# keith2018/TinyGPT

Hardware: AMD Instinct MI355X
Metric: decode tokens/sec (and % HBM roofline), Llama-3.2-1B bf16 batch=1, 1 GPU (higher is better)
Workload: dtype bf16; 1 GPU; Llama-3.2-1B bf16, batch 1 per GPU: 2048-token prefill then greedy decode (one step = one token, context 2054..3411); replicas=1, params=1235814400, graph=True

## Files before the change

__graft_entry__.py:

```python
import os
import sys

ROOT = os.path.dirname(os.path.abspath(__file__))
if ROOT not in sys.path:
    sys.path.insert(0, ROOT)


def build() -> None:
    from tinygpt_amd import build as b
    lib = b.build_lib(force=False, verbose=True)
    assert os.path.exists(lib)
    host_lib, cli = b.build_host(force=False, verbose=True)
    assert os.path.exists(host_lib) and os.path.exists(cli)
    b.build_host(force=False, verbose=True, test_hooks=True)
    b.build_kv_pool_check(force=False, verbose=True)
    b.build_splice_plan_check(force=False, verbose=True)
    b.build_dev_mem_check(force=False, verbose=True)
    b.build_row_snapshot_check(force=False, verbose=True)
    b.build_attn_worklist_check(force=False, verbose=True)
    b.build_spec_draft_check(force=False, verbose=True)
    b.build_spec_mode_check(force=False, verbose=True)
    b.build_spec_rows_check(force=False, verbose=True)
    b.build_constraint_check(force=False, verbose=True)
    from oracle.oracle_ffi import build_oracle, oracle_backend
    build_oracle()
    oracle_backend()
    import tinygpt_amd
    from tinygpt_amd.ffi import product_backend
    assert product_backend().abi_version() == 3
    print("build ok:", lib)


def smoke() -> None:
    import json
    os.environ.setdefault("OMP_NUM_THREADS", "8")
    import numpy as np
    from tinygpt_amd.desc import desc_from_hf_config
    from tinygpt_amd.ffi import GREEDY, Model, SamplerCfg, product_backend
    from oracle.oracle_ffi import OracleModel, build_oracle
    build_oracle()
    gd = os.path.join(ROOT, "tests", "golden", "llama_tiny")
    cfg = json.load(open(os.path.join(gd, "config.json")))
    g = np.load(os.path.join(gd, "golden.npz"))
    d = desc_from_hf_config(cfg, "bf16")
    gpu = Model(d, product_backend(), device=0).load_synthetic(int(g["seed"]), float(g["std"])).finalize()
    ref = OracleModel(d).load_synthetic(int(g["seed"]), float(g["std"])).finalize()
    gpu.forward(g["prompt"]); ref.forward(g["prompt"])
    a, b = gpu.logits(rounded=False), ref.logits(rounded=False)
    err = float(np.abs(a - b).max() / np.abs(b).max())
    assert err < 1e-3, f"prefill logits differ from the oracle: rel {err:.3e}"
    tg, tr = gpu.sample(GREEDY), ref.sample(GREEDY)
    dg, dr = gpu.decode(4, GREEDY), ref.decode(4, GREEDY)
# ... 13 lines not shown
```

tinygpt_amd/build.py:

```python
from __future__ import annotations

import os
import shutil
import subprocess
import sys

HERE = os.path.dirname(os.path.abspath(__file__))
CSRC = os.path.join(HERE, "csrc")
LIBDIR = os.path.join(HERE, "lib")
LIB = os.path.join(LIBDIR, "libtgx_mi355x.so")
HIPCC = shutil.which("hipcc") or "/opt/rocm/bin/hipcc"
FLAGS = ["--offload-arch=gfx950", "-O3", "-std=c++17", "-fPIC", "-shared", "-fvisibility=hidden",
         "-Wall", "-Wno-unused-function", "-DNDEBUG",
         ] + (["-mllvm", "-amdgpu-mfma-vgpr-form"] if os.environ.get("TGX_VGPR_FORM", "1") == "1" else [])


TUS = ["abi", "decode", "attn", "sampler", "prefill", "prefill_f32", "skinny"]
OBJDIR = os.path.join(LIBDIR, "obj")


def _deps():
    deps = [os.path.join(HERE, "..", "include", "tgx.h"), os.path.join(CSRC, "ctx.h"), os.path.join(CSRC, "kv_pool.h"), os.path.join(CSRC, "dev_mem.h"), os.path.join(CSRC, "row_snapshot.h"),
            os.path.join(CSRC, "splice_plan.h"), os.path.join(CSRC, "attn_worklist.h"), os.path.join(CSRC, "automaton.h")]
    kd =os.path.join(CSRC, "kernels")
    return deps + [os.path.join(kd, f) for f in sorted(os.listdir(kd))]


def build_lib(force: bool = False, verbose: bool = False, extra_flags=()):
    if os.environ.get("TGX_DISSECT") == "1":
        extra_flags = list(extra_flags) + ["-DTGX_DISSECT=1"]
    if os.environ.get("TGX_EXTRA_FLAGS"):
        extra_flags = list(extra_flags) + os.environ["TGX_EXTRA_FLAGS"].split()
    cflags = [f for f in FLAGS if f != "-shared"] + list(extra_flags)
    stamp, want = LIB + ".flags", " ".join([HIPCC] + cflags)
    same_flags = os.path.exists(stamp) and open(stamp).read() == want
    os.makedirs(OBJDIR, exist_ok=True)
    deps = _deps()
    jobs = []
    for tu in TUS:
        src, obj = os.path.join(CSRC, tu + ".hip"), os.path.join(OBJDIR, tu + ".o")
        fresh = same_flags and os.path.exists(obj) and all(os.path.getmtime(obj) >= os.path.getmtime(d) for d in deps + [src])
        if force or not fresh:
            cmd = [HIPCC] + cflags + ["-c", src, "-o", obj]
            if verbose:
                print(" ".join(cmd), file=sys.stderr)
            jobs.append((tu, subprocess.Popen(cmd)))
    failed = [tu for tu, p in jobs if p.wait() != 0]
    if failed:
        raise subprocess.CalledProcessError(1, "hipcc -c " + ", ".join(failed))
    objs = [os.path.join(OBJDIR, tu + ".o") for tu in TUS]
    if jobs or not os.path.exists(LIB) or any(os.path.getmtime(LIB) < os.path.getmtime(o) for o in objs):
        cmd = [HIPCC, "--offload-arch=gfx950", "-shared", "-fPIC", "-fvisibility=hidden"] + objs + ["-o", LIB]
        if verbose:
            print(" ".join(cmd), file=sys.stderr)
        subprocess.check_call(cmd)
    with open(stamp, "w") as f:
# ... 18 lines not shown
def _build_cpu_check(name, header, force, verbose):
    src, target = os.path.join(HERE, "..", "tests", name + ".cpp"), os.path.join(TEST_BUILD, name)
    os.makedirs(TEST_BUILD, exist_ok=True)
    if force or _stale(target, [src, header]):
        cmd = [CXX, "-std=c++17", "-O1", "-g", "-fsanitize=address,undefined", "-fno-omit-frame-pointer", "-Wall", "-Wextra", src, "-o", target]
        if verbose:
            print(" ".join(cmd), file=sys.stderr)
        subprocess.check_call(cmd)
    return target


def build_kv_pool_check(force: bool = False, verbose: bool = False):
    return _build_cpu_check("kv_pool_check", os.path.join(CSRC, "kv_pool.h"), force, verbose)


def build_splice_plan_check(force: bool = False, verbose: bool = False):
    if _stale(os.path.join(TEST_BUILD, "splice_plan_check"), [os.path.join(CSRC, "kv_pool.h")]):
        force = True
    return _build_cpu_check("splice_plan_check", os.path.join(CSRC, "splice_plan.h"), force, verbose)


def build_dev_mem_check(force: bool = False, verbose: bool = False):
    return _build_cpu_check("dev_mem_check", os.path.join(CSRC, "dev_mem.h"), force, verbose)


def build_row_snapshot_check(force: bool = False, verbose: bool = False):
    return _build_cpu_check("row_snapshot_check", os.path.join(CSRC, "row_snapshot.h"), force, verbose)


def build_attn_worklist_check(force: bool = False, verbose: bool = False):
    return _build_cpu_check("attn_worklist_check", os.path.join(CSRC, "attn_worklist.h"), force, verbose)


def build_spec_draft_check(force: bool = False, verbose: bool = False):
    return _build_cpu_check("spec_draft_check", os.path.join(HOST, "spec_draft.h"), force, verbose)


def build_spec_mode_check(force: bool = False, verbose: bool = False):
    return _build_cpu_check("spec_mode_check", os.path.join(HOST, "spec_mode.h"), force, verbose)


def build_spec_rows_check(force: bool = False, verbose: bool = False):
    return _build_cpu_check("spec_rows_check", os.path.join(HOST, "spec_mode.h"), force, verbose)


def build_constraint_check(force: bool = False, verbose: bool = False):
    if _stale(os.path.join(TEST_BUILD, "constraint_check"), [os.path.join(CSRC, "automaton.h"), os.path.join(HOST, "constraint.h")]):
        force = True
    return _build_cpu_check("constraint_check", os.path.join(HOST, "constraint.cpp"), force, verbose)


def build_host(force: bool = False, verbose: bool = False, test_hooks: bool = False):
    srcs = [os.path.join(HOST, f) for f in ("loader.cpp", "engine.cpp", "regex.cpp", "tokenizer.cpp", "constraint.cpp")]
    deps = [os.path.join(HOST, f) for f in os.listdir(HOST)] + [os.path.join(HERE, "..", "include", "tgx.h"), os.path.join(CSRC, "row_snapshot.h"), os.path.join(CSRC, "automaton.h")]
    lib, cli, flags = HOST_LIB, HOST_CLI, []
    if test_hooks:
        lib, cli, flags = HOST_TEST_LIB, HOST_TEST_CLI, ["-DTGXH_TEST_HOOKS"]
    os.makedirs(os.path.dirname(lib), exist_ok=True)
    for target, extra in ((lib, [os.path.join(HOST, "engine_c.cpp"), "-shared"]), (cli, [os.path.join(HOST, "main.cpp")])):
        if not force and not _stale(target, deps):
            continue
        cmd = [CXX] + CXXFLAGS + flags + srcs + extra + ["-o", target, "-ldl"]
        if verbose:
            print(" ".join(cmd), file=sys.stderr)
        subprocess.check_call(cmd)
    return lib, cli
# ... 7 lines not shown
```

tinygpt_amd/csrc/abi.hip:

```cpp
#include <climits>
#include "ctx.h"
#include "kernels/kv_fork.h"
#include "kernels/kv_pack.h"
#include "kernels/kv_splice.h"
#include "row_snapshot.h"
#include "splice_plan.h"
#include "automaton.h"

static std::string g_create_err;

int set_err(tgx_ctx* c, int code, const char* fmt, ...) {
  char buf[512];
  va_list ap;
  va_start(ap, fmt);
  vsnprintf(buf, sizeof buf, fmt, ap);
  va_end(ap);
  if (c) c->err = buf; else g_create_err = buf;
  return code;
}

namespace {

inline uint16_t host_f32_to_bf16(float f) {
  uint32_t u;
// ... 609 lines not shown
  if (gpt2 && d.qk_norm) return set_err(nullptr, TGX_ERR_INVALID, "gpt2 has no q/k norm");
  if (d.compute_dtype != TGX_BF16 && d.compute_dtype != TGX_F16 && d.compute_dtype != TGX_F32) return set_err(nullptr, TGX_ERR_INVALID, "unknown compute dtype %d", d.compute_dtype);
  if (d.head_dim != 64 && d.head_dim != 128) return set_err(nullptr, TGX_ERR_UNSUPPORTED, "head_dim %d (64 and 128 are built)", d.head_dim);
  if (d.heads <= 0 || d.kv_heads <= 0 || d.heads % d.kv_heads) return set_err(nullptr, TGX_ERR_INVALID, "heads %% kv_heads != 0");
  if (d.heads / d.kv_heads > 16) return set_err(nullptr, TGX_ERR_UNSUPPORTED, "GQA group size %d > 16", d.heads / d.kv_heads);
  if (d.hidden % 8 || d.inter % 8 || (d.heads * d.head_dim) % 8) return set_err(nullptr, TGX_ERR_UNSUPPORTED, "hidden/intermediate sizes must be multiples of 8");
  if (d.hidden <= 0 || d.layers <= 0 || d.inter <= 0 || d.vocab <= 0 || d.max_ctx <= 0) return set_err(nullptr, TGX_ERR_INVALID, "non-positive model dimension");
  if (d.hidden > 16384) return set_err(nullptr, TGX_ERR_UNSUPPORTED, "hidden_size %d > 16384", d.hidden);
  if (d.inter > 65536 || d.heads * d.head_dim > 16384) return set_err(nullptr, TGX_ERR_UNSUPPORTED, "projection input wider than 65536 (intermediate) / 16384 (heads * head_dim)");
  int ndev = 0;
  if (hipGetDeviceCount(&ndev) != hipSuccess || ndev <= 0) return set_err(nullptr, TGX_ERR_DEVICE, "no HIP device visible (--device mi355x needs a GPU; there is no CPU fallback)");
  if (device_ordinal < 0 || device_ordinal >= ndev) return set_err(nullptr, TGX_ERR_INVALID, "device ordinal %d out of range [0,%d)", device_ordinal, ndev);

  tgx_ctx* c = new (std::nothrow) tgx_ctx();
  if (!c) return set_err(nullptr, TGX_ERR_NOMEM, "host allocation failed");
  *out_ctx = c;
  c->d = d;
  c->gpt2 = gpt2;
  if (gpt2) { c->d.tied = 1; c->d.qkv_bias = 1; }
  if (c->d.max_batch < 1) c->d.max_batch = 1;
  c->device = device_ordinal;
  c->dt = d.compute_dtype == TGX_BF16 ? tgx::DT_BF16 : (d.compute_dtype == TGX_F16 ? tgx::DT_F16 : tgx::DT_F32);
  c->esz = d.compute_dtype == TGX_F32 ? 4 : 2;
  HIP_OK(c, hipSetDevice(device_ordinal));
  hipDeviceProp_t prop;
  HIP_OK(c, hipGetDeviceProperties(&prop, device_ordinal));
  c->num_cus = prop.multiProcessorCount > 0 ? prop.multiProcessorCount : 256;
  HIP_OK(c, hipStreamCreateWithFlags(&c->stream, hipStreamNonBlocking));
  if (const char* e = getenv("TGX_NO_GRAPH")) c->use_graph = !(e[0] == '1');
  if (const char* e = getenv("TGX_PACKED_CLASSES")) c->packed_classes = atoi(e) & 7;
  c->attn_direct_max = d.head_dim == 64 ? (d.kv_heads >= 8 ? 576 : 832) : 384;
  c->attn_direct_nw4 = d.head_dim == 64 ? 192 : 0;
  c->prefill_min_rows = d.hidden > 2048 ? 4 : 5;
  c->tune[TGX_KERNEL_DOWN].ks = d.inter >= 8192 ? 4 : 2;
  c->tune[TGX_KERNEL_QKV].ks = d.hidden >= 2048 ? 4 : 1;
  if (c->dt == tgx::DT_F32) {
    c->tune[TGX_KERNEL_GATEUP].ks = 2; c->tune[TGX_KERNEL_OPROJ].ks = 2;
    if (c->gpt2) c->tune[TGX_KERNEL_QKV].ks = 2;
  }

  const int H = d.hidden, I = d.inter, V = d.vocab, qd = d.heads * d.head_dim, kvd = d.kv_heads * d.head_dim;
  int rc;
  const size_t es = c->esz;
  if ((rc = dev_alloc(c, &c->embed, (size_t)V * H * es))) return rc;
  if (!c->d.tied && (rc = dev_alloc(c, &c->lm_head, (size_t)V * H * es))) return rc;
  if ((rc = dev_alloc(c, &c->final_norm, (size_t)H * es))) return rc;
  if (gpt2 && ((rc = dev_alloc(c, &c->wpe, (size_t)d.n_positions * H * es)) || (rc = dev_alloc(c, &c->final_norm_b, (size_t)H * es)))) return rc;
  c->L.resize((size_t)d.layers);
  for (auto& w : c->L) {
    if ((rc = dev_alloc(c, &w.in_norm, (size_t)H * es))) return rc;
    if ((rc = dev_alloc(c, &w.post_norm, (size_t)H * es))) return rc;
    if ((rc = dev_alloc(c, &w.wqkv, (size_t)(qd + 2 * kvd) * H * es))) return rc;
    if (c->d.qkv_bias && (rc = dev_alloc(c, &w.bqkv, (size_t)(qd + 2 * kvd) * es))) return rc;
    if ((rc = dev_alloc(c, &w.wo, (size_t)H * qd * es))) return rc;
    if (d.qk_norm && ((rc = dev_alloc(c, &w.q_norm, (size_t)d.head_dim * es)) || (rc = dev_alloc(c, &w.k_norm, (size_t)d.head_dim * es)))) return rc;
    if ((rc = dev_alloc(c, &w.wgu, (size_t)(gpt2 ? 1 : 2) * I * H * es))) return rc;
    if ((rc = dev_alloc(c, &w.wdown, (size_t)H * I * es))) return rc;
    if (gpt2 && ((rc = dev_alloc(c, &w.in_norm_b, (size_t)H * es)) || (rc = dev_alloc(c, &w.post_norm_b, (size_t)H * es)) || (rc = dev_alloc(c, &w.bo, (size_t)H * es)) ||
                 (rc = dev_alloc(c, &w.bfc, (size_t)I * es)) || (rc = dev_alloc(c, &w.bdown, (size_t)H * es)))) return rc;
  }
  return TGX_OK;
}

int tgx_upload(tgx_ctx* c, const char* name, const void* host, const int64_t* shape, int nd, int src_dtype) {
  if (!c || !name || !host || !shape) return c ? set_err(c, TGX_ERR_INVALID, "null argument") : TGX_ERR_INVALID;
  HIP_OK(c, hipSetDevice(c->device));
// ... 73 lines not shown
  if (c->gpt2) {
    if (!c->embed_ok) return set_err(c, TGX_ERR_STATE, "Missing key: wte.weight");
    if (!c->wpe_ok) return set_err(c, TGX_ERR_STATE, "Missing key: wpe.weight");
    if (!c->final_norm_ok || !c->final_norm_b_ok) return set_err(c, TGX_ERR_STATE, "Missing key: ln_f.%s", c->final_norm_ok ? "bias" : "weight");
    for (int l = 0; l < d.layers; l++)
      if (c->L[(size_t)l].gpt2_filled != 0xfff) return set_err(c, TGX_ERR_STATE, "Missing key in h.%d", l);
  }
  if (!c->gpt2 && !c->embed_ok) return set_err(c, TGX_ERR_STATE, "Missing key: model.embed_tokens.weight");
  if (!d.tied && !c->lm_head_ok) return set_err(c, TGX_ERR_STATE, "Missing key: lm_head.weight");
  if (!c->gpt2 && !c->final_norm_ok) return set_err(c, TGX_ERR_STATE, "Missing key: model.norm.weight");
  for (int l = 0; l < d.layers && !c->gpt2; l++) {
    const LayerW& w = c->L[(size_t)l];
    static const char* merged_names[8] = {"self_attn.q_proj.weight", "self_attn.k_proj.weight", "self_attn.v_proj.weight", "mlp.gate_proj.weight", "mlp.up_proj.weight",
                                          "self_attn.q_proj.bias", "self_attn.k_proj.bias", "self_attn.v_proj.bias"};
    for (int b = 0; b < (d.qkv_bias ? 8 : 5); b++)
      if (!(w.merged_filled & (1 << b))) return set_err(c, TGX_ERR_STATE, "Missing key: model.layers.%d.%s", l, merged_names[b]);
    if (!w.in_norm_ok || !w.post_norm_ok || !w.wo_ok || !w.wdown_ok)
      return set_err(c, TGX_ERR_STATE, "Missing key: model.layers.%d.%s", l, !w.in_norm_ok ? "input_layernorm.weight" : !w.post_norm_ok ? "post_attention_layernorm.weight" : !w.wo_ok ? "self_attn.o_proj.weight" : "mlp.down_proj.weight");
    if (d.qk_norm && (!w.q_norm_ok || !w.k_norm_ok)) return set_err(c, TGX_ERR_STATE, "Missing key: model.layers.%d.self_attn.{q,k}_norm.weight", l);
  }
  if (c->finalized) return TGX_OK;

  std::vector<float> cs, sn;
  if (c->gpt2) {
    cs.assign((size_t)d.max_ctx * (hd / 2), 1.0f);
    sn.assign((size_t)d.max_ctx * (hd / 2), 0.0f);
  } else build_rope_host(d, cs, sn);
  int rc;
  if ((rc = dev_alloc(c, &c->rope_cos, cs.size()))) return rc;
  if ((rc = dev_alloc(c, &c->rope_sin, sn.size()))) return rc;
  HIP_OK(c, hipMemcpy(c->rope_cos, cs.data(), cs.size() * 4, hipMemcpyHostToDevice));
  HIP_OK(c, hipMemcpy(c->rope_sin, sn.data(), sn.size() * 4, hipMemcpyHostToDevice));

  c->lm_grid = gemv_grid(c, (V + 1) / 2, 1, c->tune[TGX_KERNEL_LMHEAD].bpc);
  int ns = c->num_cus / d.kv_heads;
  c->attn_nsplit = ns < 1 ? 1 : (ns > 32 ? 32 : ns);
  if (c->attn_nsplit_opt > 0) c->attn_nsplit = c->attn_nsplit_opt;

  c->rows.resize((size_t)d.max_batch);
  const size_t B = (size_t)d.max_batch;
  size_t kv_elems = (size_t)d.layers * d.kv_heads * d.max_ctx * hd;
  c->kv_row_elems = kv_elems;
  size_t kv_total = B * kv_elems;
  if (c->kv_budget_tokens > 0) {
    if (c->dt == tgx::DT_F32) return set_err(c, TGX_ERR_UNSUPPORTED, "kv.budget_tokens: paged KV serves the 16-bit storage dtypes");
    c->kv_paged = true;
    c->kv.init(d.max_batch, d.max_ctx, c->kv_budget_tokens, tgx::KV_BLOCK);
    kv_total = (size_t)d.layers * c->kv.n_blocks() * d.kv_heads * tgx::KV_BLOCK * hd;
    c->kv_row_elems = 1;
    if ((rc = dev_alloc(c, &c->kv_tbl, B * (size_t)c->kv.tbl_stride()))) return rc;
    HIP_OK(c, hipMemset(c->kv_tbl, 0, B * (size_t)c->kv.tbl_stride() * 4));
  }
  c->attn_part_row = (size_t)d.heads * c->attn_nsplit * (hd + 4);
  if ((rc = dev_alloc(c, &c->slab_x, B * H))) return rc;
  if ((rc = dev_alloc(c, &c->slab_q, B * qd))) return rc;
  if ((rc = dev_alloc(c, &c->slab_kraw, B * kvd))) return rc;
  if ((rc = dev_alloc(c, &c->slab_attn, B * qd))) return rc;
  if ((rc = dev_alloc(c, &c->slab_h, B * I))) return rc;
  if ((rc = dev_alloc(c, &c->slab_logits, B * V))) return rc;
  if ((rc = dev_alloc(c, &c->slab_probs, B * V))) return rc;
  if ((rc = dev_alloc(c, &c->slab_part_val, B * c->lm_grid))) return rc;
  if ((rc = dev_alloc(c, &c->slab_part_idx, B * c->lm_grid))) return rc;
  if ((rc = dev_alloc(c, &c->slab_attn_part, B * c->attn_part_row))) return rc;
  if ((rc = dev_alloc(c, &c->slab_tok, B))) return rc;
  if ((rc = dev_alloc(c, &c->slab_pos, B))) return rc;
  if ((rc = dev_alloc(c, &c->slab_prompt, B * d.max_ctx))) return rc;
  if ((rc = dev_alloc(c, &c->slab_k, kv_total * c->esz))) return rc;
// ... 1833 lines not shown
  if (!strcmp(key, "snapshot.stage_kib")) { if (value < 1) return set_err(c, TGX_ERR_INVALID, "snapshot.stage_kib is a size in KiB (one layer of a row is always staged)"); c->snapshot_stage_kib = value; return TGX_OK; }
  if (!strcmp(key, "oproj.sliced")) { drop_step_graphs(c); c->oproj_sliced = value != 0; return TGX_OK; }
  if (!strcmp(key, "weights.packed") || !strcmp(key, "weights.packed_classes")) {
    if (c->finalized) return set_err(c, TGX_ERR_STATE, "%s is set before tgx_finalize (the packed copies are made there)", key);
    if (key[14] == '_') { if (value < 0 || value > 7) return set_err(c, TGX_ERR_INVALID, "weights.packed_classes is a mask of gate_up (1), down (2), lm_head (4)"); c->packed_classes = value; }
    else c->weights_packed = value != 0;
    return TGX_OK;
  }
  if (!strcmp(key, "kv.budget_tokens")) {
    if (c->finalized) return set_err(c, TGX_ERR_STATE, "kv.budget_tokens is set before tgx_finalize (it sizes the caches)");
    if (value < 0) return set_err(c, TGX_ERR_INVALID, "kv.budget_tokens >= 0 (0 = one max_ctx slab per row)");
    c->kv_budget_tokens = value; return TGX_OK;
  }
  if (!strcmp(key, "attn.nsplit")) {
    if (c->finalized) return set_err(c, TGX_ERR_STATE, "attn.nsplit must be set before tgx_finalize");
    if (value < 1 || value > 32) return set_err(c, TGX_ERR_INVALID, "attn.nsplit out of range");
    c->attn_nsplit_opt = value;
    return TGX_OK;
  }
  for (int i = 0; i < TGX_KERNEL_COUNT; i++) {
    const size_t n = strlen(cls_names[i]);
    if (strncmp(key, cls_names[i], n) || key[n] != '.') continue;
    if (!strcmp(key + n + 1, "ks")) {
      if (value != 1 && value != 2 && value != 4) return set_err(c, TGX_ERR_INVALID, "ks must be 1, 2 or 4");
      c->tune[i].ks = value;
      return TGX_OK;
    }
    if (!strcmp(key + n + 1, "bpc")) {
      if (value < 1 || value > 16) return set_err(c, TGX_ERR_INVALID, "bpc out of range");
      if (i == TGX_KERNEL_LMHEAD && c->finalized) return set_err(c, TGX_ERR_STATE, "lmhead.bpc must be set before tgx_finalize");
      c->tune[i].bpc = value;
      return TGX_OK;
    }
  }
  return set_err(c, TGX_ERR_INVALID, "unknown option %s", key);
}

int64_t tgx_bytes_per_token(const tgx_ctx* c, int64_t T) {
  if (!c) return -1;
  const tgx_model_desc& d = c->d;
  const int64_t H = d.hidden, I = d.inter, V = d.vocab, L = d.layers, q = (int64_t)d.heads * d.head_dim, kv = (int64_t)d.kv_heads * d.head_dim;
  const int64_t b = (int64_t)c->esz;
  if (c->gpt2) {
    const int64_t per_layer = 3 * H * H + 3 * H + H * H + H + I * H + I + H * I + H + 4 * H;
    return b * (L * per_layer + 2 * H + H + V * H) + b * 2 * L * kv * T;
  }
  const int64_t per_layer = (q + 2 * kv) * H + (d.qkv_bias ? (q + 2 * kv) : 0) + H * q + 2 * I * H + H * I + 2 * H;
  int64_t saved = 0;
  auto packed_saving = [&](const PackedMat& m, int64_t rows, int64_t cols) { if (m.P) saved += b * rows * cols - rows * (m.row_bytes + 16); };
  for (const LayerW& w : c->L) { packed_saving(w.pgu, 2 * I, H); packed_saving(w.pdown, H, I); }
  packed_saving(c->plm, V, H);
  return b * (L * per_layer + H + V * H) + b * 2 * L * kv * T - saved;
}

}
```

tinygpt_amd/csrc/ctx.h:

```cpp
#pragma once
#include <hip/hip_runtime.h>

#include <algorithm>
#include <cmath>
#include <cstdarg>
#include <cstdio>
#include <cstdlib>
#include <cstring>
#include <string>
#include <vector>

#include "../../include/tgx.h"
#include "kernels/common.h"
#include "kv_pool.h"
#include "dev_mem.h"

using tgx::bf16_t;
typedef unsigned char ebyte;

namespace tgx { struct SampScratch; struct LpRecord; struct LpRow; }

constexpr int MAX_TICKET_EVENTS = 64;
constexpr int HOST_RING = 256;

// ... 19 lines not shown
  int gpt2_filled = 0;
};

struct RowState {
  float *x = nullptr, *q = nullptr, *attn = nullptr, *h = nullptr;
  float* k_raw = nullptr;
  float* logits = nullptr;
  float* probs = nullptr;
  float* part_val = nullptr;
  int* part_idx = nullptr;
  float* attn_part = nullptr;
  int *tok = nullptr, *pos = nullptr;
  long long* prompt = nullptr;
  ebyte *kcache = nullptr, *vcache = nullptr;
  const int* tbl = nullptr;
};

struct RowHost {
  int64_t past = 0;
  bool tok = false;
  bool idle = false;
  bool nologits = false;
  char fin = 0;
  int64_t lp_count = 0;
  bool probs_ok = false; tgx_sampler_cfg probs_cfg{};
  bool probs_proc = false;
  int auto_id = -1;
  void restart(int64_t len, bool idle_, char fin_) { past = len; tok = nologits = false; idle = idle_; fin = fin_; }
};

struct Tune {
  int ks = 1;
  int bpc = 4;
};

struct Profiler {
  bool on = false;
  hipEvent_t ev[2 * 8] = {};
  int64_t launches[TGX_KERNEL_COUNT] = {};
  double ms[TGX_KERNEL_COUNT] = {};
};

struct QkvEpi { bf16_t *q_hi = nullptr, *q_lo = nullptr, *k = nullptr, *v = nullptr; int past = 0; const int* tbl = nullptr; };

struct ScoreCall {
  int top_n = 0, n_score = 0;
  const long long* ids = nullptr;
  void* host = nullptr; size_t host_bytes = 0;
};

struct EmbedCall {
  static constexpr int SLICE = 32;
  int pool = 0, normalize = 0, dims = 0;
  int n = 0;
  int cur = 0;
  std::vector<int> tab;
  int slices = 0;
  float* host_out = nullptr;
  int np(int t) const { return tab[(size_t)t * 4 + 1]; }
};

namespace tgx { struct RgSeq; struct RgItem; struct MixItem; }
struct RaggedPass {
  int n = 0, M = 0, longest = 0;
  const int *rows = nullptr, *lens = nullptr, *first = nullptr;
  const long long* ids = nullptr;
// ... 322 lines not shown
```

tinygpt_amd/csrc/decode.hip:

```cpp
#include "ctx.h"
#include "kernels/attn_decode.h"
#include "kernels/gemv.h"
#include "kernels/gemv_packed.h"
#include "kernels/oproj_sliced.h"
#include "kernels/verify.h"

int gemv_grid(const tgx_ctx* c, int units, int ks, int bpc) {
  const int upb = 4 / ks;
  const int want = (units + upb - 1) / upb;
  const int cap = c->num_cus * bpc;
  return want < cap ? want : cap;
}

static int gemv_nx(int K, int ks) { return ((K / 8) + ks * 64 - 1) / (ks * 64); }

static int gemv_auto_ks(int K, int want) {
  int ks = want;
  while (ks < 4 && gemv_nx(K, ks) > 8) ks *= 2;
  return ks;
}

static tgx::GemvArgs gemv_row(const tgx_ctx* c, tgx::GemvArgs a, int r) {
  a.x += (size_t)r * a.x_stride;
  if (a.out) a.out += (size_t)r * a.out_stride;
  if (a.q_out) a.q_out += (size_t)r * a.q_stride;
  if (a.k_raw) a.k_raw += (size_t)r * a.kraw_stride;
  if (a.k_cache) a.k_cache = (ebyte*)a.k_cache + (size_t)r * a.kv_stride * c->esz;
  if (a.v_cache) a.v_cache = (ebyte*)a.v_cache + (size_t)r * a.kv_stride * c->esz;
  if (a.pos) a.pos += r;
  if (a.blk_tbl) a.blk_tbl += (size_t)r * a.tbl_stride;
  if (a.logits) a.logits += (size_t)r * a.logits_stride;
  if (a.part_val) a.part_val += (size_t)r * a.part_stride;
  if (a.part_idx) a.part_idx += (size_t)r * a.part_stride;
  return a;
}

template <int DT, int PRO, int EPI, int NX>
static void launch_gemv_nx(tgx_ctx* c, const tgx::GemvArgs& a, int grid, int R) {
  const dim3 g(grid), b(256);
  if (R == 4) { hipLaunchKernelGGL((tgx::gemv_kernel<DT, PRO, EPI, NX, 4>), g, b, 0, c->stream, a); return; }
  if (R == 2) { hipLaunchKernelGGL((tgx::gemv_kernel<DT, PRO, EPI, NX, 2>), g, b, 0, c->stream, a); return; }
  if constexpr (DT != tgx::DT_F32 && ((PRO == tgx::PRO_RMSNORM && EPI == tgx::EPI_SILU_MUL) || (PRO == tgx::PRO_PLAIN && EPI == tgx::EPI_RESIDUAL))) {
    if (R == 1 && (a.x_acc || a.res_acc)) { hipLaunchKernelGGL((tgx::gemv_kernel<DT, PRO, EPI, NX, 1, true>), g, b, a.x_acc ? (size_t)a.K * 4 : 0, c->stream, a); return; }
  }
  for (int r = 0; r < R; r++) hipLaunchKernelGGL((tgx::gemv_kernel<DT, PRO, EPI, NX, 1>), g, b, 0, c->stream, gemv_row(c, a, r));
}

template <int PRO, int EPI, int NX>
static void launch_gemv_packed_nx(tgx_ctx* c, const tgx::GemvPackedArgs& p, int grid) {
  const dim3 g(grid), b(256);
  if constexpr (EPI != tgx::EPI_LOGITS) {
    if (p.g.x_acc || p.g.res_acc) { hipLaunchKernelGGL((tgx::gemv_packed_kernel<PRO, EPI, NX, true>), g, b, p.g.x_acc ? (size_t)p.g.K * 4 : 0, c->stream, p); return; }
  }
  hipLaunchKernelGGL((tgx::gemv_packed_kernel<PRO, EPI, NX, false>), g, b, 0, c->stream, p);
}

template <int PRO, int EPI>
static void launch_gemv_packed(tgx_ctx* c, const tgx::GemvArgs& a, const PackedMat& pk, int grid, int nx) {
  tgx::GemvPackedArgs p{};
  p.g = a; p.P = pk.P; p.rec = pk.rec; p.row_bytes = pk.row_bytes; p.e0h4 = pk.e0h4;
  switch (nx) {
    case 1: launch_gemv_packed_nx<PRO, EPI, 1>(c, p, grid); break;
    case 2: launch_gemv_packed_nx<PRO, EPI, 2>(c, p, grid); break;
    case 3: launch_gemv_packed_nx<PRO, EPI, 3>(c, p, grid); break;
    case 4: launch_gemv_packed_nx<PRO, EPI, 4>(c, p, grid); break;
    case 5: launch_gemv_packed_nx<PRO, EPI, 5>(c, p, grid); break;
    case 6: launch_gemv_packed_nx<PRO, EPI, 6>(c, p, grid); break;
    case 7: launch_gemv_packed_nx<PRO, EPI, 7>(c, p, grid); break;
    default: launch_gemv_packed_nx<PRO, EPI, 8>(c, p, grid); break;
  }
}

static int pack_matrix(tgx_ctx* c, const ebyte* W, int N, int K, int cls, int* stat_dev, PackedMat* out) {
  const int ks = gemv_auto_ks(K, c->tune[cls].ks), nx = gemv_nx(K, ks);
  if (K % 8 || K > tgx::PACKED_K_MAX || nx > 8) return TGX_OK;
  PackedMat m;
  m.ks = ks; m.row_bytes = (long long)ks * ((nx + 3) / 4) * 3072;
  int rc;
  if ((rc = dev_alloc(c, &m.P, (size_t)N * (size_t)m.row_bytes)) || (rc = dev_alloc(c, &m.rec, (size_t)N))) { dev_free(c, &m.P); return rc; }
  HIP_OK(c, hipMemsetAsync(stat_dev, 0, 4 * sizeof(int), c->stream));
  const size_t n8 = (size_t)N * K / 8;
  hipLaunchKernelGGL(tgx::packed_maxexp_kernel, dim3((unsigned)std::min<size_t>((n8 + 255) / 256, 4096)), dim3(256), 0, c->stream, reinterpret_cast<const bf16_t*>(W), n8, stat_dev);
  tgx::PackRowsArgs a{};
  a.W = reinterpret_cast<const bf16_t*>(W); a.N = N; a.K = K; a.ks = ks; a.nx = nx; a.P = m.P; a.rec = m.rec; a.row_bytes = m.row_bytes; a.stat = stat_dev;
  hipLaunchKernelGGL(tgx::pack_rows_kernel, dim3(N), dim3(64), 0, c->stream, a);
  int stat[4] = {0, 0, 0, 0};
  HIP_OK(c, hipGetLastError());
  HIP_OK(c, hipMemcpyAsync(stat, stat_dev, sizeof(stat), hipMemcpyDeviceToHost, c->stream));
  HIP_OK(c, hipStreamSynchronize(c->stream));
  c->packed_max_row_esc = std::max(c->packed_max_row_esc, stat[3]);
  if (stat[1] > 0) {
    dev_free(c, &m.P); dev_free(c, &m.rec);
    c->packed_fallbacks++;
    return TGX_OK;
  }
  const unsigned int E0h = (unsigned int)std::max((stat[0] >> 1) - 7, 0);
  m.e0h4 = E0h * 0x01010101u; m.n_esc = stat[2]; m.max_row_esc = stat[3];
  *out = m;
  c->packed_matrices++;
  return TGX_OK;
}

int pack_weights(tgx_ctx* c) {
  const tgx_model_desc& d = c->d;
  if (!c->weights_packed || c->dt != tgx::DT_BF16 || c->gpt2) return TGX_OK;
  int* stat_dev = nullptr;
  int rc = dev_alloc(c, &stat_dev, 4);
  for (size_t l = 0; l < c->L.size() && !rc; l++) {
    LayerW& w = c->L[l];
    if (c->packed_classes & 1) rc = pack_matrix(c, w.wgu, 2 * d.inter, d.hidden, TGX_KERNEL_GATEUP, stat_dev, &w.pgu);
    if (!rc && (c->packed_classes & 2) && d.inter <= 16384) rc = pack_matrix(c, w.wdown, d.hidden, d.inter, TGX_KERNEL_DOWN, stat_dev, &w.pdown);
  }
  if (!rc && (c->packed_classes & 4)) rc = pack_matrix(c, d.tied ? c->embed : c->lm_head, d.vocab, d.hidden, TGX_KERNEL_LMHEAD, stat_dev, &c->plm);
  dev_free(c, &stat_dev);
  return rc;
}

template <int PRO, int EPI>
static void launch_gemv(tgx_ctx* c, tgx::GemvArgs a, int cls, int R, const PackedMat* pk = nullptr) {
  const Tune& tn = c->tune[cls];
  a.dbg = ((c->debug_gemv >> (8 + cls)) & 1) ? (c->debug_gemv & 15) : 0;
  if (!a.ldw) a.ldw = a.K;
  a.ks = gemv_auto_ks(a.K, tn.ks);
  while (R > 1 && a.ks < 4 && gemv_nx(a.K, a.ks) > 4) a.ks *= 2;
  if (R == 2 && cls == TGX_KERNEL_GATEUP && a.ks == 1 && gemv_nx(a.K, 1) == 4) a.ks = 2;
  const int grid = (EPI == tgx::EPI_LOGITS) ? c->lm_grid : gemv_grid(c, a.units, a.ks, tn.bpc);
  const int nx = gemv_nx(a.K, a.ks);
  if constexpr ((PRO == tgx::PRO_RMSNORM && (EPI == tgx::EPI_SILU_MUL || EPI == tgx::EPI_LOGITS)) || (PRO == tgx::PRO_PLAIN && EPI == tgx::EPI_RESIDUAL)) {
    if (pk && pk->P && R == 1 && pk->ks == a.ks && a.ldw == a.K && !a.dbg) { launch_gemv_packed<PRO, EPI>(c, a, *pk, grid, nx); return; }
  }
  if constexpr (PRO == tgx::PRO_LAYERNORM || EPI == tgx::EPI_GELU) {
    TGX_DT_SWITCH(c->dt, switch (nx) {
      case 1: launch_gemv_nx<DT, PRO, EPI, 1>(c, a, grid, R); break;
      case 2: launch_gemv_nx<DT, PRO, EPI, 2>(c, a, grid, R); break;
      case 3: launch_gemv_nx<DT, PRO, EPI, 3>(c, a, grid, R); break;
      default: launch_gemv_nx<DT, PRO, EPI, 4>(c, a, grid, R); break;
    })
  } else {
    TGX_DT_SWITCH(c->dt, switch (nx) {
      case 1: launch_gemv_nx<DT, PRO, EPI, 1>(c, a, grid, R); break;
      case 2: launch_gemv_nx<DT, PRO, EPI, 2>(c, a, grid, R); break;
      case 3: launch_gemv_nx<DT, PRO, EPI, 3>(c, a, grid, R); break;
      case 4: launch_gemv_nx<DT, PRO, EPI, 4>(c, a, grid, R); break;
      case 5: launch_gemv_nx<DT, PRO, EPI, 5>(c, a, grid, R); break;
      case 6: launch_gemv_nx<DT, PRO, EPI, 6>(c, a, grid, R); break;
      case 7: launch_gemv_nx<DT, PRO, EPI, 7>(c, a, grid, R); break;
      default: launch_gemv_nx<DT, PRO, EPI, 8>(c, a, grid, R); break;
    })
  }
}

static void fill_strides(const tgx_ctx* c, tgx::GemvArgs& a) {
  const tgx_model_desc& d = c->d;
  a.x_stride = 0; a.out_stride = 0;
  a.q_stride = (long long)d.heads * d.head_dim; a.kraw_stride = (long long)d.kv_heads * d.head_dim;
  a.kv_stride = (long long)c->kv_row_elems; a.logits_stride = d.vocab; a.part_stride = c->lm_grid;
  a.act16 = c->act16;
}

static bool qk_fused(const tgx_ctx* c, long long kv_stride) { return c->d.qk_norm && c->d.head_dim == 128 && kv_stride != 0 && c->qk_fuse; }

bool oproj_sliced_ok(const tgx_ctx* c, int R, long long kv_stride) {
// ... 233 lines not shown
```

tinygpt_amd/csrc/kernels/gemv_packed.h:

```cpp
#pragma once
#include "gemv.h"

namespace tgx {

constexpr int PACKED_ESC = 4;
constexpr int PACKED_K_MAX = 32768;

struct PackedQuad { u32x4 l01, l23, nb; };

struct GemvPackedArgs {
  GemvArgs g;
  const unsigned char* P;
  const u32x4* rec;
  long long row_bytes;
  unsigned int e0h4;
};

typedef float f32x2 __attribute__((ext_vector_type(2)));

__device__ __forceinline__ f32x2 pk_fma_x0(f32x2 w, f32x2 x, f32x2 acc) {
  asm("v_pk_fma_f32 %0, %1, %2, %0 op_sel_hi:[1,0,1]" : "+v"(acc) : "v"(w), "v"(x));
  return acc;
}
__device__ __forceinline__ f32x2 pk_fma_x1(f32x2 w, f32x2 x, f32x2 acc) {
// ... 36 lines not shown
  static_assert(PRO == PRO_PLAIN || PRO == PRO_RMSNORM, "packed forms: plain or RMSNorm prologue");
  static_assert(EPI == EPI_SILU_MUL || EPI == EPI_RESIDUAL || EPI == EPI_LOGITS, "packed forms: gate_up, down, lm_head");
  const GemvArgs& a = pa.g;
  const int n_wg = (int)gridDim.x;
  __shared__ float ps[4][2];
  __shared__ float sv[1][4];
  __shared__ int si[1][4];

  const int lane = threadIdx.x & 63, wv = threadIdx.x >> 6;
  const int KS = a.ks, UPB = 4 / KS;
  const int slot = wv / KS, kpart = wv - slot * KS;
  const int nchunk = a.K >> 3;
  const int per = ((nchunk + KS * 64 - 1) / (KS * 64)) * 64;
  const int c_begin = min(kpart * per, nchunk), c_end = min(c_begin + per, nchunk);
  const int stride = n_wg * UPB;
  const int c0_u = __builtin_amdgcn_readfirstlane(c_begin);

  int cidx[NX];
  bool cok[NX];
#pragma unroll
  for (int j = 0; j < NX; j++) {
    const int c = c_begin + lane + 64 * j;
    cok[j] = c < c_end;
    cidx[j] = cok[j] ? c : max(c_end - 1, 0);
  }

  const size_t lane_off = (size_t)kpart * NQ * 3072 + (size_t)lane * 16;
  PackedQuad wa[NQ], wb[NQ], na[NQ], nb[NQ];
  u32x4 ea, eb, nea = {}, neb = {};
  auto load_unit = [&](int ub, PackedQuad* ta, PackedQuad* tb, u32x4& ra_rec, u32x4& rb_rec) {
    const int u = min(ub + slot, a.units - 1);
    int ra, rb; bool v;
    unit_rows<EPI>(a, u, ra, rb, v);
    ra_rec = pa.rec[ra]; rb_rec = pa.rec[rb];
    const unsigned char* pra = pa.P + (size_t)ra * pa.row_bytes + lane_off;
    const unsigned char* prb = pa.P + (size_t)rb * pa.row_bytes + lane_off;
#pragma unroll
    for (int q = 0; q < NQ; q++) {
      const u32x4* qa = reinterpret_cast<const u32x4*>(pra + (size_t)q * 3072);
      const u32x4* qb = reinterpret_cast<const u32x4*>(prb + (size_t)q * 3072);
      ta[q].l01 = load_nt(qa); ta[q].l23 = load_nt(qa + 64); ta[q].nb = load_nt(qa + 128);
      tb[q].l01 = load_nt(qb); tb[q].l23 = load_nt(qb + 64); tb[q].nb = load_nt(qb + 128);
    }
  };
  auto rec_uniform = [](const u32x4 v) {
    return u32x4{(unsigned int)__builtin_amdgcn_readfirstlane((int)v[0]), (unsigned int)__builtin_amdgcn_readfirstlane((int)v[1]),
                 (unsigned int)__builtin_amdgcn_readfirstlane((int)v[2]), (unsigned int)__builtin_amdgcn_readfirstlane((int)v[3])};
  };

  float xr[NX][8];
  auto load_x = [&]() {
    const f32x4* xg = reinterpret_cast<const f32x4*>(a.x);
#pragma unroll
    for (int j = 0; j < NX; j++) {
      f32x4 v0 = xg[2 * cidx[j]], v1 = xg[2 * cidx[j] + 1];
      if (!cok[j]) { v0 = f32x4{0.f, 0.f, 0.f, 0.f}; v1 = v0; }
#pragma unroll
      for (int t = 0; t < 4; t++) { xr[j][t] = v0[t]; xr[j][4 + t] = v1[t]; }
    }
  };
  ulonglong2 xacc0[(XACC && PRO == PRO_RMSNORM) ? 4 : 1];
  if constexpr (XACC && PRO == PRO_RMSNORM) {
    const ulonglong2* ag = reinterpret_cast<const ulonglong2*>(a.x_acc + (size_t)min((int)threadIdx.x, nchunk - 1) * 8);
#pragma unroll
    for (int q = 0; q < 4; q++) xacc0[q] = ag[q];
    __builtin_amdgcn_sched_barrier(0);
  }
// ... 169 lines not shown
}

__global__ __launch_bounds__(256) void packed_maxexp_kernel(const bf16_t* W, size_t n8, int* stat) {
  int m = 0;
  for (size_t i = (size_t)blockIdx.x * 256 + threadIdx.x; i < n8; i += (size_t)gridDim.x * 256) {
    const u32x4 v = reinterpret_cast<const u32x4*>(W)[i];
#pragma unroll
    for (int t = 0; t < 4; t++) {
      const int e0 = (v[t] >> 7) & 0xff, e1 = (v[t] >> 23) & 0xff;
      if (e0 < 255) m = max(m, e0);
      if (e1 < 255) m = max(m, e1);
    }
  }
#pragma unroll
  for (int o = 32; o > 0; o >>= 1) m = max(m, __shfl_xor(m, o, 64));
  if ((threadIdx.x & 63) == 0) atomicMax(stat, m);
}

__device__ __forceinline__ bool packed_is_escape(unsigned int bits, int E0h) {
  const int e = (int)((bits >> 7) & 0xff), d = (e >> 1) - E0h;
  return d < 0 || d > 7 || e == 0 || e == 255;
}

struct PackRowsArgs {
  const bf16_t* W;
  int N, K, ks, nx;
  unsigned char* P;
  u32x4* rec;
  long long row_bytes;
  int* stat;
};

__global__ __launch_bounds__(64) void pack_rows_kernel(const PackRowsArgs a) {
  __shared__ unsigned int ent[PACKED_ESC];
  const int row = blockIdx.x, lane = threadIdx.x;
  const int E0h = max((a.stat[0] >> 1) - 7, 0);
  const bf16_t* w = a.W + (size_t)row * a.K;
  if (lane < PACKED_ESC) ent[lane] = 0xffffffffu;
  __syncthreads();
  int cnt = 0;
  for (int k0 = 0; k0 < a.K; k0 += 64) {
    const int k = k0 + lane;
    unsigned int bits = 0; bool esc = false;
    if (k < a.K) { bits = w[k]; esc = packed_is_escape(bits, E0h); }
    const unsigned long long bal = __ballot(esc);
    const int p = cnt + __popcll(bal & ((1ull << lane) - 1ull));
    if (esc && p < PACKED_ESC) ent[p] = ((unsigned int)k << 16) | bits;
    cnt += __popcll(bal);
  }
  __syncthreads();
  if (lane == 0) {
    a.rec[row] = u32x4{ent[0], ent[1], ent[2], ent[3]};
    if (cnt > PACKED_ESC) atomicAdd(a.stat + 1, 1);
    if (cnt) { atomicAdd(a.stat + 2, cnt); atomicMax(a.stat + 3, cnt); }
  }
  const int nchunk = a.K >> 3, nq = (a.nx + 3) / 4;
  const int per = ((nchunk + a.ks * 64 - 1) / (a.ks * 64)) * 64;
  for (int p = 0; p < a.ks; p++) {
    const int c_begin = min(p * per, nchunk), c_end = min(c_begin + per, nchunk);
    for (int q = 0; q < nq; q++) {
      unsigned int L[8], Nb[4];
#pragma unroll
      for (int jj = 0; jj < 4; jj++) {
        const int j = 4 * q + jj, c = c_begin + lane + 64 * j;
        L[2 * jj] = 0; L[2 * jj + 1] = 0; Nb[jj] = 0;
        if (j < a.nx && c < c_end) {
          const u32x4 v = reinterpret_cast<const u32x4*>(w)[c];
          unsigned int lo[8], n[8];
#pragma unroll
          for (int t = 0; t < 8; t++) {
            const unsigned int bits = (v[t >> 1] >> (16 * (t & 1))) & 0xffffu;
            const bool esc = packed_is_escape(bits, E0h);
            lo[t] = esc ? 0u : (bits & 0xffu);
            n[t] = esc ? 0u : (((bits >> 12) & 8u) | (((bits >> 8) & 0x7fu) - (unsigned int)E0h));
          }
          L[2 * jj] = lo[0] | (lo[1] << 8) | (lo[2] << 16) | (lo[3] << 24);
          L[2 * jj + 1] = lo[4] | (lo[5] << 8) | (lo[6] << 16) | (lo[7] << 24);
          unsigned int nn = 0;
#pragma unroll
          for (int t = 0; t < 4; t++) nn |= (n[t] << (8 * t)) | (n[4 + t] << (8 * t + 4));
          Nb[jj] = nn;
        }
      }
      u32x4* dst = reinterpret_cast<u32x4*>(a.P + (size_t)row * a.row_bytes + ((size_t)p * nq + q) * 3072) + lane;
      dst[0] = u32x4{L[0], L[1], L[2], L[3]};
      dst[64] = u32x4{L[4], L[5], L[6], L[7]};
      dst[128] = u32x4{Nb[0], Nb[1], Nb[2], Nb[3]};
    }
  }
}
// ... 3 lines not shown
```

Measured before the change: 1590 tokens/s.

## Store packed escape records per K-split and add separate packed GEMV grid sizing

After: 1621 tokens/s (median of 6 runs). 1.02x the previous value.

```diff
diff --git a/__graft_entry__.py b/__graft_entry__.py
--- a/__graft_entry__.py
+++ b/__graft_entry__.py
@@ -18,6 +18,7 @@
     b.build_dev_mem_check(force=False, verbose=True)
     b.build_row_snapshot_check(force=False, verbose=True)
     b.build_attn_worklist_check(force=False, verbose=True)
+    b.build_gemv_grid_check(force=False, verbose=True)
     b.build_spec_draft_check(force=False, verbose=True)
     b.build_spec_mode_check(force=False, verbose=True)
     b.build_spec_rows_check(force=False, verbose=True)
diff --git a/tinygpt_amd/build.py b/tinygpt_amd/build.py
--- a/tinygpt_amd/build.py
+++ b/tinygpt_amd/build.py
@@ -21,7 +21,7 @@
 
 def _deps():
     deps = [os.path.join(HERE, "..", "include", "tgx.h"), os.path.join(CSRC, "ctx.h"), os.path.join(CSRC, "kv_pool.h"), os.path.join(CSRC, "dev_mem.h"), os.path.join(CSRC, "row_snapshot.h"),
-            os.path.join(CSRC, "splice_plan.h"), os.path.join(CSRC, "attn_worklist.h"), os.path.join(CSRC, "automaton.h")]
+            os.path.join(CSRC, "splice_plan.h"), os.path.join(CSRC, "attn_worklist.h"), os.path.join(CSRC, "automaton.h"), os.path.join(CSRC, "gemv_grid.h")]
     kd =os.path.join(CSRC, "kernels")
     return deps + [os.path.join(kd, f) for f in sorted(os.listdir(kd))]
 
@@ -106,6 +106,10 @@
     return _build_cpu_check("attn_worklist_check", os.path.join(CSRC, "attn_worklist.h"), force, verbose)
 
 
+def build_gemv_grid_check(force: bool = False, verbose: bool = False):
+    return _build_cpu_check("gemv_grid_check", os.path.join(CSRC, "gemv_grid.h"), force, verbose)
+
+
 def build_spec_draft_check(force: bool = False, verbose: bool = False):
     return _build_cpu_check("spec_draft_check", os.path.join(HOST, "spec_draft.h"), force, verbose)
 
diff --git a/tinygpt_amd/csrc/abi.hip b/tinygpt_amd/csrc/abi.hip
--- a/tinygpt_amd/csrc/abi.hip
+++ b/tinygpt_amd/csrc/abi.hip
@@ -665,6 +665,7 @@
   c->attn_direct_max = d.head_dim == 64 ? (d.kv_heads >= 8 ? 576 : 832) : 384;
   c->attn_direct_nw4 = d.head_dim == 64 ? 192 : 0;
   c->prefill_min_rows = d.hidden > 2048 ? 4 : 5;
+  c->tune[TGX_KERNEL_GATEUP].packed_bpc = 3;
   c->tune[TGX_KERNEL_DOWN].ks = d.inter >= 8192 ? 4 : 2;
   c->tune[TGX_KERNEL_QKV].ks = d.hidden >= 2048 ? 4 : 1;
   if (c->dt == tgx::DT_F32) {
@@ -804,7 +805,8 @@
   HIP_OK(c, hipMemcpy(c->rope_cos, cs.data(), cs.size() * 4, hipMemcpyHostToDevice));
   HIP_OK(c, hipMemcpy(c->rope_sin, sn.data(), sn.size() * 4, hipMemcpyHostToDevice));
 
-  c->lm_grid = gemv_grid(c, (V + 1) / 2, 1, c->tune[TGX_KERNEL_LMHEAD].bpc);
+  const bool lm_packed = c->weights_packed && (c->packed_classes & 4) && c->dt == tgx::DT_BF16 && !c->gpt2;
+  c->lm_grid = gemv_grid(c, (V + 1) / 2, 1, lm_packed ? c->tune[TGX_KERNEL_LMHEAD].packed_bpc : c->tune[TGX_KERNEL_LMHEAD].bpc);
   int ns = c->num_cus / d.kv_heads;
   c->attn_nsplit = ns < 1 ? 1 : (ns > 32 ? 32 : ns);
   if (c->attn_nsplit_opt > 0) c->attn_nsplit = c->attn_nsplit_opt;
@@ -2704,6 +2706,12 @@
       c->tune[i].bpc = value;
       return TGX_OK;
     }
+    if (!strcmp(key + n + 1, "packed_bpc") && (i == TGX_KERNEL_GATEUP || i == TGX_KERNEL_DOWN || i == TGX_KERNEL_LMHEAD)) {
+      if (value < 1 || value > 16) return set_err(c, TGX_ERR_INVALID, "packed_bpc out of range");
+      if (i == TGX_KERNEL_LMHEAD && c->finalized) return set_err(c, TGX_ERR_STATE, "lmhead.packed_bpc must be set before tgx_finalize");
+      c->tune[i].packed_bpc = value;
+      return TGX_OK;
+    }
   }
   return set_err(c, TGX_ERR_INVALID, "unknown option %s", key);
 }
@@ -2719,7 +2727,7 @@
   }
   const int64_t per_layer = (q + 2 * kv) * H + (d.qkv_bias ? (q + 2 * kv) : 0) + H * q + 2 * I * H + H * I + 2 * H;
   int64_t saved = 0;
-  auto packed_saving = [&](const PackedMat& m, int64_t rows, int64_t cols) { if (m.P) saved += b * rows * cols - rows * (m.row_bytes + 16); };
+  auto packed_saving = [&](const PackedMat& m, int64_t rows, int64_t cols) { if (m.P) saved += b * rows * cols - rows * (m.row_bytes + 16 * m.ks); };
   for (const LayerW& w : c->L) { packed_saving(w.pgu, 2 * I, H); packed_saving(w.pdown, H, I); }
   packed_saving(c->plm, V, H);
   return b * (L * per_layer + H + V * H) + b * 2 * L * kv * T - saved;
diff --git a/tinygpt_amd/csrc/ctx.h b/tinygpt_amd/csrc/ctx.h
--- a/tinygpt_amd/csrc/ctx.h
+++ b/tinygpt_amd/csrc/ctx.h
@@ -75,6 +75,7 @@
 struct Tune {
   int ks = 1;
   int bpc = 4;
+  int packed_bpc = 4;
 };
 
 struct Profiler {
diff --git a/tinygpt_amd/csrc/decode.hip b/tinygpt_amd/csrc/decode.hip
--- a/tinygpt_amd/csrc/decode.hip
+++ b/tinygpt_amd/csrc/decode.hip
@@ -1,16 +1,12 @@
 #include "ctx.h"
+#include "gemv_grid.h"
 #include "kernels/attn_decode.h"
 #include "kernels/gemv.h"
 #include "kernels/gemv_packed.h"
 #include "kernels/oproj_sliced.h"
 #include "kernels/verify.h"
 
-int gemv_grid(const tgx_ctx* c, int units, int ks, int bpc) {
-  const int upb = 4 / ks;
-  const int want = (units + upb - 1) / upb;
-  const int cap = c->num_cus * bpc;
-  return want < cap ? want : cap;
-}
+int gemv_grid(const tgx_ctx* c, int units, int ks, int bpc) { return tgx::gemv_grid_plan(units, 4 / ks, c->num_cus * bpc).grid; }
 
 static int gemv_nx(int K, int ks) { return ((K / 8) + ks * 64 - 1) / (ks * 64); }
 
@@ -77,7 +73,7 @@
   PackedMat m;
   m.ks = ks; m.row_bytes = (long long)ks * ((nx + 3) / 4) * 3072;
   int rc;
-  if ((rc = dev_alloc(c, &m.P, (size_t)N * (size_t)m.row_bytes)) || (rc = dev_alloc(c, &m.rec, (size_t)N))) { dev_free(c, &m.P); return rc; }
+  if ((rc = dev_alloc(c, &m.P, (size_t)N * (size_t)m.row_bytes)) || (rc = dev_alloc(c, &m.rec, (size_t)N * (size_t)ks))) { dev_free(c, &m.P); return rc; }
   HIP_OK(c, hipMemsetAsync(stat_dev, 0, 4 * sizeof(int), c->stream));
   const size_t n8 = (size_t)N * K / 8;
   hipLaunchKernelGGL(tgx::packed_maxexp_kernel, dim3((unsigned)std::min<size_t>((n8 + 255) / 256, 4096)), dim3(256), 0, c->stream, reinterpret_cast<const bf16_t*>(W), n8, stat_dev);
@@ -127,7 +123,10 @@
   const int grid = (EPI == tgx::EPI_LOGITS) ? c->lm_grid : gemv_grid(c, a.units, a.ks, tn.bpc);
   const int nx = gemv_nx(a.K, a.ks);
   if constexpr ((PRO == tgx::PRO_RMSNORM && (EPI == tgx::EPI_SILU_MUL || EPI == tgx::EPI_LOGITS)) || (PRO == tgx::PRO_PLAIN && EPI == tgx::EPI_RESIDUAL)) {
-    if (pk && pk->P && R == 1 && pk->ks == a.ks && a.ldw == a.K && !a.dbg) { launch_gemv_packed<PRO, EPI>(c, a, *pk, grid, nx); return; }
+    if (pk && pk->P && R == 1 && pk->ks == a.ks && a.ldw == a.K && !a.dbg) {
+      launch_gemv_packed<PRO, EPI>(c, a, *pk, (EPI == tgx::EPI_LOGITS) ? grid : gemv_grid(c, a.units, a.ks, tn.packed_bpc), nx);
+      return;
+    }
   }
   if constexpr (PRO == tgx::PRO_LAYERNORM || EPI == tgx::EPI_GELU) {
     TGX_DT_SWITCH(c->dt, switch (nx) {
diff --git a/tinygpt_amd/csrc/gemv_grid.h b/tinygpt_amd/csrc/gemv_grid.h
--- /dev/null
+++ b/tinygpt_amd/csrc/gemv_grid.h
@@ -0,0 +1,19 @@
+#pragma once
+
+namespace tgx {
+
+struct GemvGrid {
+  int grid;
+  int rounds;
+};
+
+inline GemvGrid gemv_grid_plan(int units, int upb, int cap) {
+  if (units < 1) units = 1;
+  if (upb < 1) upb = 1;
+  if (cap < 1) cap = 1;
+  const int want = (units + upb - 1) / upb;
+  const int grid = want < cap ? want : cap;
+  return GemvGrid{grid, (want + grid - 1) / grid};
+}
+
+}
diff --git a/tinygpt_amd/csrc/kernels/gemv_packed.h b/tinygpt_amd/csrc/kernels/gemv_packed.h
--- a/tinygpt_amd/csrc/kernels/gemv_packed.h
+++ b/tinygpt_amd/csrc/kernels/gemv_packed.h
@@ -92,7 +92,7 @@
     const int u = min(ub + slot, a.units - 1);
     int ra, rb; bool v;
     unit_rows<EPI>(a, u, ra, rb, v);
-    ra_rec = pa.rec[ra]; rb_rec = pa.rec[rb];
+    ra_rec = pa.rec[(size_t)ra * KS + kpart]; rb_rec = pa.rec[(size_t)rb * KS + kpart];
     const unsigned char* pra = pa.P + (size_t)ra * pa.row_bytes + lane_off;
     const unsigned char* prb = pa.P + (size_t)rb * pa.row_bytes + lane_off;
 #pragma unroll
@@ -328,30 +328,33 @@
 };
 
 __global__ __launch_bounds__(64) void pack_rows_kernel(const PackRowsArgs a) {
-  __shared__ unsigned int ent[PACKED_ESC];
+  __shared__ unsigned int ent[4][PACKED_ESC];
   const int row = blockIdx.x, lane = threadIdx.x;
   const int E0h = max((a.stat[0] >> 1) - 7, 0);
   const bf16_t* w = a.W + (size_t)row * a.K;
-  if (lane < PACKED_ESC) ent[lane] = 0xffffffffu;
+  const int nchunk = a.K >> 3, nq = (a.nx + 3) / 4;
+  const int per = ((nchunk + a.ks * 64 - 1) / (a.ks * 64)) * 64;
+  if (lane < 4 * PACKED_ESC) ent[lane / PACKED_ESC][lane % PACKED_ESC] = 0xffffffffu;
   __syncthreads();
-  int cnt = 0;
+  int cnt = 0, part = 0, pcnt = 0, pmax = 0;
   for (int k0 = 0; k0 < a.K; k0 += 64) {
+    const int kp = (k0 >> 3) / per;
+    if (kp != part) { part = kp; pcnt = 0; }
     const int k = k0 + lane;
     unsigned int bits = 0; bool esc = false;
     if (k < a.K) { bits = w[k]; esc = packed_is_escape(bits, E0h); }
     const unsigned long long bal = __ballot(esc);
-    const int p = cnt + __popcll(bal & ((1ull << lane) - 1ull));
-    if (esc && p < PACKED_ESC) ent[p] = ((unsigned int)k << 16) | bits;
-    cnt += __popcll(bal);
+    const int p = pcnt + __popcll(bal & ((1ull << lane) - 1ull));
+    if (esc && p < PACKED_ESC) ent[part][p] = ((unsigned int)k << 16) | bits;
+    const int n = __popcll(bal);
+    cnt += n; pcnt += n; pmax = max(pmax, pcnt);
   }
   __syncthreads();
+  if (lane < a.ks) a.rec[(size_t)row * a.ks + lane] = u32x4{ent[lane][0], ent[lane][1], ent[lane][2], ent[lane][3]};
   if (lane == 0) {
-    a.rec[row] = u32x4{ent[0], ent[1], ent[2], ent[3]};
-    if (cnt > PACKED_ESC) atomicAdd(a.stat + 1, 1);
+    if (pmax > PACKED_ESC) atomicAdd(a.stat + 1, 1);
     if (cnt) { atomicAdd(a.stat + 2, cnt); atomicMax(a.stat + 3, cnt); }
   }
-  const int nchunk = a.K >> 3, nq = (a.nx + 3) / 4;
-  const int per = ((nchunk + a.ks * 64 - 1) / (a.ks * 64)) * 64;
   for (int p = 0; p < a.ks; p++) {
     const int c_begin = min(p * per, nchunk), c_end = min(c_begin + per, nchunk);
     for (int q = 0; q < nq; q++) {
```
